# GuoleiSun/VSS-CFFM

Measured on AMD Instinct MI355X. Metric: clips/sec (fwd+bwd) CFFM-B1 480x480 T=4 hot path (CFFA+CFM, decoder_focal depth 2), higher is better.
Workload: dtype f32 in/out, f32 accumulate; MFMA operands: split-bf16 (hi+lo, ~2^-17) in the Linear GEMMs, f16 in QK^T/AV

## Files before the change

vss_cffm_amd/csrc/cffa_kernels.h:

```cpp
#pragma once
#include "cffm_common.h"

__device__ __forceinline__ void transpose_body(const float* __restrict__ src, float* __restrict__ dst,
                                               int rows, int cols, long src_bs, long dst_bs,
                                               const float* __restrict__ addend, int add_mod, int add_skip,
                                               float* __restrict__ copy_dst, int bx, int by, int bz) {
    __shared__ float tile[64][65];
    const int r0 = by * 64, c0 = bx * 64;
    const float* s = src + (long)bz * src_bs;
    float* d = dst + (long)bz * dst_bs;
    const int q = threadIdx.x & 15, p = threadIdx.x >> 4;
    const bool vin = (cols % 4 == 0) && (src_bs % 4 == 0) && (((uintptr_t)src & 15) == 0);
    const bool vout = (rows % 4 == 0) && (dst_bs % 4 == 0) && (((uintptr_t)dst & 15) == 0) && (((uintptr_t)addend & 15) == 0);
    const float* ad = (addend && (bz % add_mod) != add_skip) ? addend + (long)bz * dst_bs : nullptr;
    float* cp = (copy_dst && (bz % add_mod) != add_skip) ? copy_dst + (long)bz * src_bs : nullptr;
#pragma unroll
    for (int k = 0; k < 4; ++k) {
        const int r = r0 + p + 16 * k, c = c0 + 4 * q;
        f32x4 v = (f32x4){0.f, 0.f, 0.f, 0.f};
        if (r < rows) {
            if (vin && c + 3 < cols) {
                v = *(const f32x4*)(s + (long)r * cols + c);
                if (cp) *(f32x4*)(cp + (long)r * cols + c) = v;
            } else
                for (int e = 0; e < 4; ++e)
                    if (c + e < cols) { v[e] = s[(long)r * cols + c + e]; if (cp) cp[(long)r * cols + c + e] = v[e]; }
// ... 8 lines not shown
        f32x4 v;
#pragma unroll
        for (int e = 0; e < 4; ++e) v[e] = tile[cl][4 * q + e];
        if (c < cols) {
            if (vout && r + 3 < rows) *(f32x4*)(d + (long)c * rows + r) = ad ? v + *(const f32x4*)(ad + (long)c * rows + r) : v;
            else
                for (int e = 0; e < 4; ++e)
                    if (r + e < rows) d[(long)c * rows + r + e] = v[e] + (ad ? ad[(long)c * rows + r + e] : 0.f);
        }
    }
}
__global__ void __launch_bounds__(256) k_transpose(const float* __restrict__ src, float* __restrict__ dst,
                                                    int rows, int cols, long src_bs, long dst_bs,
                                                    const float* __restrict__ addend, int add_mod, int add_skip,
                                                    float* __restrict__ copy_dst = nullptr) {
    transpose_body(src, dst, rows, cols, src_bs, dst_bs, addend, add_mod, add_skip, copy_dst, blockIdx.x, blockIdx.y, blockIdx.z);
}

__device__ __forceinline__ float bil_tap(int r, int p) {
    if (p == r) return (11.f - 2.f * r) * (1.f / 12.f);
    if (p == r + 1) return (1.f + 2.f * r) * (1.f / 12.f);
    return 0.f;
}

__device__ __forceinline__ void cell_geom(int g, int& grp, int& u, int& v, int& wsg) {
    if (g == 0) { grp = 0; u = v = 0; wsg = 7; }
    else if (g == 1) { grp = 1; u = v = 0; wsg = 7; }
    else if (g < 6) { grp = 2; u = (g - 2) >> 1; v = (g - 2) & 1; wsg = 3; }
    else { grp = 3; u = (g - 6) / 3; v = (g - 6) % 3; wsg = 2; }
}

// ... 170 lines not shown

#define LNP_RSTRIDE 1216
#define LNP_TAIL_TGT (CFFM_WA + 1)
#define LNP_TAIL_REF (14 * CFFM_WA + 3)
#ifndef LNB_SPLIT
#define LNB_SPLIT 4
#endif
#ifndef LNB_WAVES
#define LNB_WAVES 4
#endif
#define LNB_THREADS (64 * LNB_WAVES)
#define LNB_PIX ((CFFM_WA + LNB_SPLIT * LNB_WAVES - 1) / (LNB_SPLIT * LNB_WAVES))

__device__ __forceinline__ float dot4(f32x4 a, f32x4 b) { return a[0] * b[0] + a[1] * b[1] + a[2] * b[2] + a[3] * b[3]; }

__global__ void __launch_bounds__(LNB_THREADS) k_ln_pool_bwd_tgt(Geo G, const float* __restrict__ x_tgt, long tgt_bs,
                                                                 const float* __restrict__ gamma, const float* __restrict__ beta,
                                                                 const float* __restrict__ M, const float* __restrict__ mean_in,
                                                                 const float* __restrict__ rstd_in, const float* __restrict__ dzall,
                                                                 const float* __restrict__ dres, float* __restrict__ dx_tgt, long dtgt_bs,
                                                                 float* __restrict__ rec) {
    __shared__ float red[LNB_WAVES][2][CFFM_C];
    __shared__ float sdM[CFFM_WA];
    __shared__ float sbs;
    const int s = blockIdx.x % LNB_SPLIT, wb = blockIdx.x / LNB_SPLIT;
    const int w = wb % G.nW, b = wb / G.nW;
    const int wy = w / G.gx, wx = w % G.gx;
    const int lane = threadIdx.x & 63, wave = wave_uniform(threadIdx.x >> 6);
    const float* xf = x_tgt + (long)b * tgt_bs;
    float* dxf = dx_tgt + (long)b * dtgt_bs;
    if (threadIdx.x < CFFM_WA) sdM[threadIdx.x] = 0.f;
    f32x4 xr[LNB_PIX], dzr[LNB_PIX], addr[LNB_PIX];
    float mur[LNB_PIX], rsr[LNB_PIX], m0[LNB_PIX];
#pragma unroll
    for (int k = 0; k < LNB_PIX; ++k) {
        const int i = s + LNB_SPLIT * (wave + LNB_WAVES * k);
        const int y = 7 * wy + i / 7, x = 7 * wx + i % 7;
        xr[k] = dzr[k] = addr[k] = (f32x4){0.f, 0.f, 0.f, 0.f};
        mur[k] = rsr[k] = m0[k] = 0.f;
        if (i < CFFM_WA && y < G.H0 && x < G.W0) {
// ... 26 lines not shown
        const f32x4 z = xh * gm + bt;
        const f32x4 dz = dzr[k] + m0[k] * dp;
        const float dm = wave_sum_hi(dot4(dp, z));
        if (lane == 63) sdM[i] = dm;
        ag += dz * xh;
        ab += dz;
        const f32x4 gz = dz * gm;
        const float m1 = wave_sum(gz[0] + gz[1] + gz[2] + gz[3]) * (1.f / CFFM_C);
        const float m2 = wave_sum(dot4(gz, xh)) * (1.f / CFFM_C);
        const f32x4 dx = (gz - m1 - xh * m2) * rs + addr[k];
        *(f32x4*)(dxf + pix * CFFM_C + 4 * lane) = dx;
    }
    *(f32x4*)(&red[wave][0][4 * lane]) = ag;
    *(f32x4*)(&red[wave][1][4 * lane]) = ab;
    __syncthreads();
    float* r = rec + (long)blockIdx.x * LNP_RSTRIDE;
    for (int e = threadIdx.x; e < 2 * CFFM_C; e += LNB_THREADS) {
        const int which = e / CFFM_C, ch = e % CFFM_C;
        float t = red[0][which][ch];
#pragma unroll
        for (int q = 1; q < LNB_WAVES; ++q) t += red[q][which][ch];
        r[e] = t;
    }
    if (threadIdx.x < CFFM_WA) r[2 * CFFM_C + threadIdx.x] = sdM[threadIdx.x];
    if (threadIdx.x == CFFM_WA) r[2 * CFFM_C + CFFM_WA] = sbs;
}

#define RB_MAXD 4
struct CffaRefBlocks {
    int n;
    const float* gamma[RB_MAXD];
    const float* beta[RB_MAXD];
    const float* M[RB_MAXD];
    const float* dzall[RB_MAXD];
    float* rec[RB_MAXD];
};
#define RB_LDS_BLOCK (14 * CFFM_C + 2 * 14 * CFFM_WA)
__host__ __device__ constexpr int cffa_ref_lds(int D) {
    return 4 * ((D * RB_LDS_BLOCK > LNB_WAVES * D * 2 * CFFM_C + 14 * D * CFFM_WA ? D * RB_LDS_BLOCK : LNB_WAVES * D * 2 * CFFM_C + 14 * D * CFFM_WA) + 4 * D + 4);
}
// ... 51 lines not shown
                    const float dm = wave_sum_hi(dot4(dp, z));
                    if (lane == 63) sdM[c * CFFM_WA + i] = dm;
                }
            ag[d] += dz * xh;
            ab[d] += dz;
            gz += dz * gm[d];
        }
        const float m1 = wave_sum(gz[0] + gz[1] + gz[2] + gz[3]) * (1.f / CFFM_C);
        const float m2 = wave_sum(dot4(gz, xh)) * (1.f / CFFM_C);
        const f32x4 dx = (gz - m1 - xh * m2) * rs + R.add[k];
        *(f32x4*)(dxf + pix * CFFM_C + 4 * lane) = dx;
    }
}

template <int D, bool ACC>
__global__ void __launch_bounds__(LNB_THREADS) k_ln_pool_bwd_ref(Geo G, const float* __restrict__ x_ref, long ref_bs, CffaRefBlocks Bk,
                                                                 const float* __restrict__ mean_in, const float* __restrict__ rstd_in,
                                                                 float* __restrict__ dx_ref, long dref_bs) {
    CFFM_DYN_SMEM(smem);
    float* sP = (float*)smem;
    float* sMm = sP + D * 14 * CFFM_C;
    float* red = (float*)smem;
    constexpr int body = D * (14 * CFFM_C + 14 * CFFM_WA), redn = LNB_WAVES * D * 2 * CFFM_C;
    float* sdM = (float*)smem + (body > redn ? body : redn);
    float* sbs = sdM + D * 14 * CFFM_WA;
    const int s = blockIdx.x % LNB_SPLIT, wb = blockIdx.x / LNB_SPLIT;
    const int w = wb % G.nW, b = wb / G.nW;
    const int wy = w / G.gx, wx = w % G.gx;
    const int lane = threadIdx.x & 63, wave = wave_uniform(threadIdx.x >> 6);
    for (int e = threadIdx.x; e < D * 14 * CFFM_WA; e += LNB_THREADS) {
        const int d = e / (14 * CFFM_WA), r = e % (14 * CFFM_WA);
        sMm[e] = Bk.M[d][CFFM_WA + r];
        sdM[e] = 0.f;
    }
    for (int r = wave; r < D * 14; r += LNB_WAVES) {
        const int d = r / 14, c = r % 14;
        *(f32x4*)(sP + r * CFFM_C + 4 * lane) = *(const f32x4*)(Bk.dzall[d] + ((long)b * G.RC + cell_row(G, wy, wx, 1 + c)) * CFFM_C + 4 * lane);
    }
    f32x4 gm[D], bt[D], ag[D], ab[D];
#pragma unroll
    for (int d = 0; d < D; ++d) {
// ... 23 lines not shown
    RefRows Ra, Rb;
    ln_pool_ref_load<ACC>(Ra, G, xb, dxb, mb, rb, s, wy, wx, lane, wave);
    ln_pool_ref_load<ACC>(Rb, G, xb + fr, dxb + fr, mb + G.HW, rb + G.HW, s, wy, wx, lane, wave);
    ln_pool_bwd_ref_frame<1, D>(G, Ra, dxb, sP, sMm, sdM, gm, bt, ag, ab, 1, s, wy, wx, lane, wave);
    ln_pool_ref_load<ACC>(Ra, G, xb + 2 * fr, dxb + 2 * fr, mb + 2 * G.HW, rb + 2 * G.HW, s, wy, wx, lane, wave);
    ln_pool_bwd_ref_frame<4, D>(G, Rb, dxb + fr, sP, sMm, sdM, gm, bt, ag, ab, 2, s, wy, wx, lane, wave);
    ln_pool_bwd_ref_frame<9, D>(G, Ra, dxb + 2 * fr, sP, sMm, sdM, gm, bt, ag, ab, 6, s, wy, wx, lane, wave);
    __syncthreads();
#pragma unroll
    for (int d = 0; d < D; ++d) {
        *(f32x4*)(red + ((wave * D + d) * 2 + 0) * CFFM_C + 4 * lane) = ag[d];
        *(f32x4*)(red + ((wave * D + d) * 2 + 1) * CFFM_C + 4 * lane) = ab[d];
    }
    __syncthreads();
    for (int d = 0; d < D; ++d) {
        float* r = Bk.rec[d] + (long)blockIdx.x * LNP_RSTRIDE;
        for (int e = threadIdx.x; e < 2 * CFFM_C; e += LNB_THREADS) {
            float t = red[(d * 2) * CFFM_C + e];
#pragma unroll
            for (int q = 1; q < LNB_WAVES; ++q) t += red[((q * D + d) * 2) * CFFM_C + e];
            r[e] = t;
        }
        for (int e = threadIdx.x; e < LNP_TAIL_REF; e += LNB_THREADS)
            r[2 * CFFM_C + e] = e < 14 * CFFM_WA ? sdM[d * 14 * CFFM_WA + e] : sbs[d * 4 + (e - 14 * CFFM_WA)];
    }
}
```

vss_cffm_amd/csrc/cffm_hip.hip:

```cpp
#include "cfm_attn_kernels.h"
#include "clip_kernels.h"
#include "rowops_kernels.h"
#include "gtc_kernels.h"
#include "gemm.h"
#include "segfuse_kernels.h"
#include "segloss_kernels.h"
#include "headfuse_kernels.h"
#include "kmeans_kernels.h"

#include <stdarg.h>
#include <stdio.h>

#include "../../include/cffm_hip.h"

static thread_local char g_err[512] = "";

static int fail(int code, const char* fmt, ...) {
    va_list ap;
    va_start(ap, fmt);
    vsnprintf(g_err, sizeof(g_err), fmt, ap);
    va_end(ap);
    return code;
}
#define CHECK_LAUNCH(name)                                                                        \
// ... 513 lines not shown
static float* g_redbuf[2] = {nullptr, nullptr};
static size_t g_red_floats_[2] = {0, 0};
static int g_red_parity = 0;
#define g_red g_redbuf[g_red_parity]
#define g_red_floats g_red_floats_[g_red_parity]
static struct { bool active; size_t bump; RedJobs jobs; } g_rq = {false, 0, {}};
static void redq_launch(RedJobs& J, hipStream_t st) {
    if (J.njob == 1) {
        CFFM_LAUNCH(k_reduce_records, ((J.total[0] + 63) / 64), (1024), 0, st, J.part[0], J.nblk[0], J.stride[0], J.total[0], J.segs[0]);
    } else if (J.njob > 1) {
        CFFM_LAUNCH(k_reduce_records_multi, ((unsigned)J.blk_end[J.njob - 1]), (1024), 0, st, J);
    }
    J.njob = 0;
}
static void redq_flush(hipStream_t st) { redq_launch(g_rq.jobs, st); }
struct RedScope {
    hipStream_t st;
    explicit RedScope(hipStream_t s) : st(s) { g_red_parity ^= 1; g_rq.active = true; g_rq.bump = 0; g_rq.jobs.njob = 0; }
    void finish() { redq_flush(st); g_rq.active = false; }
    void finish_on(hipStream_t other) { redq_flush(other); g_rq.active = false; }
    ~RedScope() { g_rq.active = false; g_rq.jobs.njob = 0; }
};
static float* red_scratch(size_t nfloats, hipStream_t st) {
    if (!g_rq.active) return lib_scratch(nfloats);
    nfloats = (nfloats + 63) / 64 * 64;
    if (g_rq.bump + nfloats > g_red_floats) {
#ifndef CFFM_EMU
        (void)hipDeviceSynchronize();
#endif
        redq_flush(st);
// ... 97 lines not shown
                             float* dx_ref, long dref_bs, int accum, hipStream_t st) {
    constexpr int lds = cffa_ref_lds(D);
#ifndef CFFM_EMU
    static bool granted = false;
    if (!granted && lds > 64 * 1024) {
        if (hipFuncSetAttribute((const void*)k_ln_pool_bwd_ref<D, false>, hipFuncAttributeMaxDynamicSharedMemorySize, lds) != hipSuccess ||
            hipFuncSetAttribute((const void*)k_ln_pool_bwd_ref<D, true>, hipFuncAttributeMaxDynamicSharedMemorySize, lds) != hipSuccess) return -1;
        granted = true;
    }
#endif
    if (accum) CFFM_LAUNCH((k_ln_pool_bwd_ref<D, true>), ((unsigned)cffa_rows(g)), (LNB_THREADS), lds, st, to_geo(g), x_ref, ref_bs, Bk, mean, rstd, dx_ref, dref_bs);
    else CFFM_LAUNCH((k_ln_pool_bwd_ref<D, false>), ((unsigned)cffa_rows(g)), (LNB_THREADS), lds, st, to_geo(g), x_ref, ref_bs, Bk, mean, rstd, dx_ref, dref_bs);
    return 0;
}
}
static int ln_pool_bwd_ref(const cffm_geom* g, const float* x_ref, long ref_bs, const CffaRefBlocks& Bk, const float* mean, const float* rstd,
                           float* dx_ref, long dref_bs, int accum, void* stream) {
    PROF(ST_LN_POOL_BWD_REF);
    hipStream_t st = (hipStream_t)stream;
    int rc = -1;
    switch (Bk.n) {
        case 1: rc = ln_pool_bwd_ref_d<1>(g, x_ref, ref_bs, Bk, mean, rstd, dx_ref, dref_bs, accum, st); break;
        case 2: rc = ln_pool_bwd_ref_d<2>(g, x_ref, ref_bs, Bk, mean, rstd, dx_ref, dref_bs, accum, st); break;
        case 3: rc = ln_pool_bwd_ref_d<3>(g, x_ref, ref_bs, Bk, mean, rstd, dx_ref, dref_bs, accum, st); break;
        case 4: rc = ln_pool_bwd_ref_d<4>(g, x_ref, ref_bs, Bk, mean, rstd, dx_ref, dref_bs, accum, st); break;
        default: break;
    }
    REQUIRE(!rc, "ln_pool_bwd_ref: bad block count %d or LDS grant failed", Bk.n);
    CHECK_LAUNCH("ln_pool_bwd_ref");
    return 0;
}
static void job_add(RedJobs& J, const float* part, int nblk, int stride, int total, const RedSegs& segs, hipStream_t st) {
    if (J.njob == RED_MAXJOB) redq_launch(J, st);
    const int j = J.njob++;
    J.part[j] = part; J.nblk[j] = nblk; J.stride[j] = stride; J.total[j] = total; J.segs[j] = segs;
    J.blk_end[j] = (j ? J.blk_end[j - 1] : 0) + (total + 63) / 64;
// ... 23 lines not shown
    if (g_scr4) { (void)hipDeviceSynchronize(); (void)hipFree(g_scr4); }
    if (hipMalloc((void**)&g_scr4, nfloats * sizeof(float)) != hipSuccess) g_scr4 = nullptr;
#endif
    g_scr4_floats = g_scr4 ? nfloats : 0;
    return g_scr4;
}
struct CffaSlot { float* dzall; float* rec; float* dM; };
static int cffa_slot(const cffm_geom* g, int slot, int nslots, CffaSlot* o) {
    const long a = up((long)g->B * g->RC * CFFM_C), b = up(2 * cffa_rows(g) * LNP_RSTRIDE), c = up(CFFM_NCELL * CFFM_WA);
    float* base = lib_scratch4((size_t)(a + b + c) * nslots);
    REQUIRE(base && slot >= 0 && slot < nslots, "cffa: scratch allocation failed");
    float* p = base + (a + b + c) * slot;
    o->dzall = p; o->rec = p + a; o->dM = p + a + b;
    return 0;
}
static int cffa_finish(const cffm_geom* g, int nslots, const cffm_block_params* params, const cffm_block_grads* grads, int first, int last,
                       const float* ws0, long ws_stride, const float* x_ref, long ref_bs, float* dx_ref, long dref_bs, int accum, void* stream,
                       RedJobs* extra = nullptr) {
    cffm_block_ws L;
    cffm_block_ws_layout(g, &L);
    hipStream_t st = (hipStream_t)stream;
    const long rows = cffa_rows(g);
    static_assert(PMB_MAXD == RB_MAXD, "one pooling-matrix launch per reference launch");
    for (int hi = first; hi >= last; hi -= RB_MAXD) {
        const int n = hi - last + 1 < RB_MAXD ? hi - last + 1 : RB_MAXD;
        CffaRefBlocks Bk;
        PoolWGN pw;
        RedJobs J;
        Bk.n = n; J.njob = 0;
        for (int d = 0; d < RB_MAXD; ++d) {
            const int i = hi - (d < n ? d : 0);
            CffaSlot S;
            TRY(cffa_slot(g, i, nslots, &S));
            Bk.gamma[d] = params[i].norm1_w; Bk.beta[d] = params[i].norm1_b; Bk.M[d] = ws0 + i * ws_stride + L.M;
            Bk.dzall[d] = S.dzall; Bk.rec[d] = S.rec + rows * LNP_RSTRIDE;
            pw.dM[d] = S.dM;
            for (int q = 0; q < 4; ++q) { pw.gw[d].w[q] = grads[i].pool_w[q]; pw.gw[d].b[q] = g_grad_pads ? grads[i].pool_b[q] : nullptr; }
        }
        const float* ws = ws0 + (long)hi * ws_stride;
        TRY(ln_pool_bwd_ref(g, x_ref, ref_bs, Bk, ws + L.mean1, ws + L.rstd1, dx_ref, dref_bs, accum || hi != first, stream));
        for (int d = 0; d < n; ++d) {
            const int i = hi - d;
            CffaSlot S;
            TRY(cffa_slot(g, i, nslots, &S));
            cffa_jobs(J, S.rec, rows, grads[i].norm1_w, grads[i].norm1_b, S.dM, grads[i].pool_b, st);
        }
        if (extra && hi - RB_MAXD < last) {
            for (int j = 0; j < extra->njob; ++j) job_add(J, extra->part[j], extra->nblk[j], extra->stride[j], extra->total[j], extra->segs[j], st);
            extra->njob = 0;
        }
        redq_launch(J, st);
        CHECK_LAUNCH("cffa reductions");
        {
            PROF(ST_POOLMAT);
            CFFM_LAUNCH(k_pool_matrix_bwd_n, (111, n), (64), 0, st, pw);
            CHECK_LAUNCH("pool_matrix_bwd");
        }
    }
    return 0;
}

int cffm_bias_assemble(const float* own, const float* ring, const float* const pool[4], float* bias, void* biasH, void* stream) {
    PROF(ST_BIAS_ASM);
    BiasTables t;
    t.own = own; t.ring = ring;
    for (int i = 0; i < 4; ++i) t.pool[i] = pool[i];
    const int n = CFFM_HEADS * CFFM_NQ_PAD * CFFM_NKEY_PAD;
    CFFM_LAUNCH(k_bias_assemble, ((n + 255) / 256), (256), 0, (hipStream_t)stream, t, bias, (h16*)biasH);
    CHECK_LAUNCH("bias_assemble");
    return 0;
}

// ... 629 lines not shown
                                   p->proj_b, p->fc1_b, p->fc2_b, p->norm2_w, p->norm2_b, ws + L.x1, nullptr, ws + L.mean2, ws + L.rstd2, ws + L.hraw,
                                   nullptr, ws + L.x2, ws + L.ao_t, ws + L.z2, ws + L.act, NP, stream));
        else
        TRY(cffm_mlp_fwd(ws + L.ao, x_tgt, tgt_bs, g->HW, wf + 768 * 256, wf + 768 * 256 + 256 * 256, wf + 768 * 256 + 256 * 256 + 1024 * 256,
                         p->proj_b, p->fc1_b, p->fc2_b, p->norm2_w, p->norm2_b, ws + L.x1, ws + L.z2, ws + L.mean2, ws + L.rstd2, ws + L.hraw,
                         ws + L.act, ws + L.x2, NP, stream));
        CHECK_LAUNCH("block_forward");
    }
    (void)scratch;
    return 0;
}

static int block_backward_impl(const cffm_geom* g, const cffm_block_params* p, const cffm_block_grads* gr,
                               const float* x_ref, long ref_bs, const float* x_tgt, long tgt_bs, const int* key_src,
                               const int* q_dst, const int* inv_ptr, const int* inv_idx, const float* ws, const float* dout,
                               float* dx_tgt, long dtgt_bs, float* scratch, int defer, int par, int slot, int nslots, void* stream);
#ifndef CFFM_EMU
static struct { bool has; RedJobs jobs; int parity; } g_tail = {false, {}, 0};
static int tail_flush(hipStream_t st) {
    if (!g_tail.has) return 0;
    g_tail.has = false;
    hipStream_t s3 = side_fork_take(st, 3);
    (void)hipStreamWaitEvent(s3, g_side.tail_order, 0);
    redq_launch(g_tail.jobs, s3);
    CHECK_LAUNCH("block_backward reductions");
    if (s3 != st) {
        side_record(s3, st, g_side.tail_done[g_tail.parity]);
        g_side.tail_pending[g_tail.parity] = true;
    }
    return 0;
}
// ... 6 lines not shown
    for (int i = 0; i < 2; ++i) g_side.dw_pending[i] = g_side.bias_pending[i] = g_side.tail_pending[i] = false;
#endif
}
int cffm_block_backward(const cffm_geom* g, const cffm_block_params* p, const cffm_block_grads* gr,
                        const float* x_ref, long ref_bs, const float* x_tgt, long tgt_bs, const int* key_src,
                        const int* q_dst, const int* inv_ptr, const int* inv_idx, const float* ws, const float* dout,
                        float* dx_ref, long dref_bs, int accum_ref, float* dx_tgt, long dtgt_bs, float* scratch, void* stream) {
    REQUIRE(x_ref && dx_ref, "block_backward: null");
    TRY(block_backward_impl(g, p, gr, x_ref, ref_bs, x_tgt, tgt_bs, key_src, q_dst, inv_ptr, inv_idx, ws, dout, dx_tgt, dtgt_bs, scratch, 0, 0, 0, 1,
                            stream));
    return cffa_finish(g, 1, p, gr, 0, 0, ws, 0, x_ref, ref_bs, dx_ref, dref_bs, accum_ref, stream);
}
static int block_backward_impl(const cffm_geom* g, const cffm_block_params* p, const cffm_block_grads* gr,
                               const float* x_ref, long ref_bs, const float* x_tgt, long tgt_bs, const int* key_src,
                               const int* q_dst, const int* inv_ptr, const int* inv_idx, const float* ws, const float* dout,
                               float* dx_tgt, long dtgt_bs, float* scratch, int defer, int par, int slot, int nslots, void* stream) {
    REQUIRE(g && p && gr && ws && dout && scratch, "block_backward: null");
    cffm_block_ws L;
    cffm_block_ws_layout(g, &L);
    const Scratch S = scratch_layout(g);
    const long NR = (long)g->B * g->RC, NP = (long)g->B * g->HW;
    par = (defer && par) ? 1 : 0;
    const long altb = S.alt, altact = altb + up(NP * CFFM_C), altqkv = altact + up((NP + 31) / 32 * 32 * CFFM_HID), altbias = altqkv + up(NR * 768);
    float* dx1 = scratch + (par ? altb : S.b);
    float* dz2 = scratch + S.dz2;
    float* dao = scratch + S.dao;
    float* dact = scratch + (par ? altact : S.dact);
    float* dqkv = scratch + (par ? altqkv : S.dqkv);
    const long NP32 = (NP + 31) / 32 * 32;
    float* dout_t = scratch + S.tf + (par ? S.tf_stride : 0);
    float* dx1_t = dout_t + up(NP32 * CFFM_C);
// ... 114 lines not shown
            const cffm_wgrad wgb[2] = {wg_qkv, wg_proj};
            const GemmTNPre preb[2] = {{0, 1, nullptr}, {0, 0, nullptr}};
            {
                void* stream = stream_b;
                PROF(ST_GEMM); PROF2(ST_G_DW);
                REQUIRE(!dw_group(wgb, preb, 2, sb, 320, dw_group_launched), "block_backward: weight-gradient gemm failed");
            }
            PROF(ST_ATTN_BWD);
            s1 = sb;
            TRY(attn_bwd_bias_sum(dbp, ng, dbiasT, (void*)s1));
            TRY(cffm_bias_scatter(dbiasT, gr->rpb_own, gr->rpb_ring, gr->rpb_pool, (void*)s1));
        }
        return 0;
    };
    const bool side_late = stream_dw && one_group;
    if (!side_late) TRY(side_b());
    if (!side_late && (!one_group || dx_tgt == dout)) side_join(sa, st, 0);
#ifndef CFFM_EMU
    if (g_side.dw_pending[par ^ 1] && g_side.dw_dout[par ^ 1] == dx_tgt) {
        side_wait(st, g_side.dw_done[par ^ 1]);
        g_side.dw_pending[par ^ 1] = false;
    }
#endif
    TRY(ln_pool_bwd_tgt(g, x_tgt, tgt_bs, p->norm1_w, p->norm1_b, ws + L.M, ws + L.mean1, ws + L.rstd1, dzall, dx1, dx_tgt, dtgt_bs, cffa.rec,
                        stream));
    if (side_late) TRY(side_b());
#ifndef CFFM_EMU
    if (defer && sb != st && s1 != st && g_side.on) {
        if (g_tail.has) TRY(tail_flush(st));
        side_fork_mark(st, 3);
        if (s1 != sb) side_order(s1, sb);
        (void)hipEventRecord(g_side.tail_order, sb);
        g_tail.has = true; g_tail.jobs = g_rq.jobs; g_tail.parity = g_red_parity;
        g_rq.jobs.njob = 0; g_rq.active = false;
        g_side.dw_pending[par] = true;
        g_side.dw_dout[par] = dout;
        side_record(s1, st, g_side.bias_done[par]);
        g_side.bias_pending[par] = true;
        return 0;
    }
#endif
// ... 451 lines not shown
    REQUIRE(hipMemcpyAsync(y_rows, blk0 + (long)(depth - 1) * L.total + L.x2, (size_t)g->B * img * sizeof(float), hipMemcpyDeviceToDevice,
                           (hipStream_t)stream) == hipSuccess, "layer_forward_rows: copy failed");
#endif
    return 0;
}
int cffm_layer_backward_rows(const cffm_geom* g, int depth, const cffm_block_params* params, const cffm_block_grads* grads,
                             const float* x_rows, const float* dy_rows, float* dx_rows, const int* key_src, const int* q_dst,
                             const int* inv_ptr, const int* inv_idx, const float* saved, float* scratch, void* stream) {
    REQUIRE(g && params && grads && x_rows && dy_rows && dx_rows && saved && scratch && depth >= 1, "layer_backward_rows: bad arguments");
    cffm_block_ws L;
    cffm_block_ws_layout(g, &L);
    const Scratch S = scratch_layout(g);
    const long HW = g->HW, img = HW * CFFM_C;
    const float* blk0 = saved + up((long)g->B * 4 * img);
    tail_reset();
    for (int i = depth - 1; i >= 0; --i) {
        const float* ws = blk0 + (long)i * L.total;
        const float* tgt = (i == 0) ? x_rows + 3 * img : blk0 + (long)(i - 1) * L.total + L.x2;
        const long tgt_bs = (i == 0) ? 4 * img : img;
        float* dtgt = (i == 0) ? dx_rows + 3 * img : scratch + (((depth - i) & 1) ? S.a2 : S.a);
        const long dtgt_bs = (i == 0) ? 4 * img : img;
        const float* dout = (i == depth - 1) ? dy_rows : scratch + (((depth - 1 - i) & 1) ? S.a2 : S.a);
        TRY(block_backward_impl(g, &params[i], &grads[i], x_rows, 4 * img, tgt, tgt_bs, key_src, q_dst, inv_ptr, inv_idx, ws, dout, dtgt, dtgt_bs,
                                scratch, 1, (depth - 1 - i) & 1, i, depth, stream));
    }
    RedJobs* tail_jobs = nullptr;
#ifndef CFFM_EMU
    if (g_tail.has) {
        g_tail.has = false;
        tail_jobs = &g_tail.jobs;
    }
#endif
    TRY(cffa_finish(g, depth, params, grads, depth - 1, 0, blk0, L.total, x_rows, 4 * img, dx_rows, 4 * img, 0, stream, tail_jobs));
    side_join_all((hipStream_t)stream);
    return 0;
}

static int layer_forward_impl(const cffm_geom* g, int depth, const cffm_block_params* params, const float* x_nchw,
                              float* y_tgt_nchw, long y_bs, float* y_full, const int* key_src, const int* q_dst, float* saved,
                              float* scratch, void* stream) {
    REQUIRE(g && params && x_nchw && y_tgt_nchw && saved && scratch && depth >= 1, "layer_forward: bad arguments");
    cffm_block_ws L;
    cffm_block_ws_layout(g, &L);
    const long HW = g->HW, img = HW * CFFM_C;
    float* xs = saved;
    float* blk0 = saved + up((long)g->B * 4 * img);
    hipStream_t st = (hipStream_t)stream;
    side_init(st);
// ... 192 lines not shown
                               const int* q_dst, const int* inv_ptr, const int* inv_idx, const float* saved, float* scratch,
                               int first_block, int last_block, void* stream) {
    REQUIRE(g && params && grads && dy_tgt_nchw && dx_nchw && saved && scratch && depth >= 1, "layer_backward: bad arguments");
    REQUIRE(first_block < depth && last_block >= 0 && first_block >= last_block, "layer_backward: bad block range %d..%d of %d", first_block,
            last_block, depth);
    cffm_block_ws L;
    cffm_block_ws_layout(g, &L);
    const Scratch S = scratch_layout(g);
    const long HW = g->HW, img = HW * CFFM_C;
    const float* xs = saved;
    const float* blk0 = saved + up((long)g->B * 4 * img);
    float* dxs = scratch + S.dxs;
    REQUIRE(dy_bs >= img, "layer_backward: dy batch stride %ld < %ld", dy_bs, img);
    if (first_block == depth - 1) TRY(cffm_transpose(dy_tgt_nchw, scratch + S.a, g->B, CFFM_C, (int)HW, dy_bs, img, stream));
    tail_reset();
    for (int i = first_block; i >= last_block; --i) {
        const float* ws = blk0 + (long)i * L.total;
        const float* tgt = (i == 0) ? xs + 3 * img : blk0 + (long)(i - 1) * L.total + L.x2;
        const long tgt_bs = (i == 0) ? 4 * img : img;
        float* dcur = scratch + (((depth - 1 - i) & 1) ? S.a2 : S.a);
        float* dtgt = (i == 0) ? dxs + 3 * img : scratch + (((depth - i) & 1) ? S.a2 : S.a);
        const long dtgt_bs = (i == 0) ? 4 * img : img;
        TRY(block_backward_impl(g, &params[i], &grads[i], xs, 4 * img, tgt, tgt_bs, key_src, q_dst, inv_ptr, inv_idx, ws, dcur, dtgt, dtgt_bs, scratch,
                                1, (depth - 1 - i) & 1, i, depth, stream));
    }
    RedJobs* tail_jobs = nullptr;
#ifndef CFFM_EMU
    if (last_block == 0 && g_tail.has) {
        g_tail.has = false;
        tail_jobs = &g_tail.jobs;
    }
#endif
    TRY(cffa_finish(g, depth, params, grads, first_block, last_block, blk0, L.total, xs, 4 * img, dxs, 4 * img, first_block != depth - 1, stream, tail_jobs));
    if (last_block == 0) TRY(transpose_add(dxs, dx_nchw, g->B * 4, (int)HW, CFFM_C, img, img, dy_full, 4, 3, stream));
    TRY(tail_flush((hipStream_t)stream));
    side_join_all((hipStream_t)stream);
    return 0;
}
int cffm_layer_backward_range(const cffm_geom* g, int depth, const cffm_block_params* params, const cffm_block_grads* grads,
                              const float* dy_tgt_nchw, long dy_bs, float* dx_nchw, const int* key_src, const int* q_dst,
                              const int* inv_ptr, const int* inv_idx, const float* saved, float* scratch, int first_block,
                              int last_block, void* stream) {
    return layer_backward_impl(g, depth, params, grads, dy_tgt_nchw, dy_bs, nullptr, dx_nchw, key_src, q_dst, inv_ptr, inv_idx, saved,
                               scratch, first_block, last_block, stream);
}
int cffm_layer_backward_full(const cffm_geom* g, int depth, const cffm_block_params* params, const cffm_block_grads* grads,
                             const float* dy_full_nchw, float* dx_nchw, const int* key_src, const int* q_dst, const int* inv_ptr,
                             const int* inv_idx, const float* saved, float* scratch, int first_block, int last_block, void* stream) {
    REQUIRE(g && dy_full_nchw && dy_full_nchw != dx_nchw, "layer_backward_full: bad arguments");
// ... 84 lines not shown
```

vss_cffm_amd/csrc/rowops_kernels.h:

```cpp
#pragma once
#include "cffm_common.h"
#include "cffa_kernels.h"
#include "panel_kernels.h"

struct BiasTables {
    const float* own;
    const float* ring;
    const float* pool[4];
};
struct BiasTablesG {
    float* own;
    float* ring;
    float* pool[4];
};

__device__ __forceinline__ int bias_locate(int h, int q, int n, int& off) {
    const int qi = q / 7, qj = q % 7;
    if (n < 49) {
        const int ki = n / 7, kj = n % 7;
        off = ((qi - ki + 6) * 13 + (qj - kj + 6)) * CFFM_HEADS + h;
        return 0;
    }
    if (n < 181) {
        off = (h * 49 + q) * 132 + (n - 49);
// ... 68 lines not shown
    if (a.pack == 2) return;
    long e = (long)(bx - a.nbias - 1) * 256 + threadIdx.x;
    long off = 0;
#pragma unroll
    for (int k = 0; k < 4; ++k) {
        if (e >= off && e < off + n4[k]) ((f32x4*)a.w_s[d])[e] = split4_pack(((const f32x4*)a.w[d][k])[e - off]);
        off += n4[k];
    }
}
__global__ void __launch_bounds__(256) k_param_prep(PrepArgs a) { param_prep_body(a, blockIdx.x, blockIdx.y); }
struct TrArgs { const float* src; float* dst; int rows, cols; long src_bs, dst_bs; int add_mod, add_skip; float* copy_dst; int gx, gy, gz; };
__global__ void __launch_bounds__(256) k_transpose_prep(TrArgs T, PrepArgs a, int pnx) {
    const int nt = T.gx * T.gy * T.gz;
    int b = blockIdx.x;
    if (b < nt) {
        transpose_body(T.src, T.dst, T.rows, T.cols, T.src_bs, T.dst_bs, nullptr, T.add_mod, T.add_skip, T.copy_dst, b % T.gx, (b / T.gx) % T.gy,
                       b / (T.gx * T.gy));
        return;
    }
    b -= nt;
    param_prep_body(a, b % pnx, b / pnx);
}

__global__ void __launch_bounds__(256) k_bias_scatter(const float* __restrict__ dbiasT, BiasTablesG g) {
    const int e = blockIdx.x * 256 + threadIdx.x;
    const int n_own = 169 * CFFM_HEADS, n_ring = CFFM_HEADS * 49 * 132;
    if (e < n_ring) {
        const int n = e % 132, q = (e / 132) % 49, h = e / (132 * 49);
        g.ring[e] = dbiasT[((long)h * CFFM_NKEY_PAD + 49 + n) * CFFM_NQ_PAD + q];
    }
    if (blockIdx.x * 256 + 255 < n_ring) return;
    const int j = (e - n_ring) & 15;
// ... 135 lines not shown
struct RedJobs {
    int njob;
    int blk_end[RED_MAXJOB];
    const float* part[RED_MAXJOB];
    int nblk[RED_MAXJOB], stride[RED_MAXJOB], total[RED_MAXJOB];
    RedSegs segs[RED_MAXJOB];
};
__global__ void __launch_bounds__(1024) k_reduce_records_multi(RedJobs J) {
    __shared__ float red[64][64];
    int blk = blockIdx.x, j = 0;
#pragma unroll
    for (int q = 0; q < RED_MAXJOB - 1; ++q)
        if (q + 1 < J.njob && blk >= J.blk_end[q]) j = q + 1;
    if (j > 0) blk -= J.blk_end[j - 1];
    reduce_records_body(J.part[j], J.nblk[j], J.stride[j], J.total[j], J.segs[j], blk, red);
}

#define COLSUM_ROWS 32
__global__ void __launch_bounds__(256) k_colsum_partial(const float* __restrict__ a, long nrows, int ncol, float* __restrict__ part) {
    const long r0 = (long)blockIdx.x * COLSUM_ROWS;
    for (int c4 = threadIdx.x; c4 < ncol / 4; c4 += 256) {
        f32x4 acc = (f32x4){0.f, 0.f, 0.f, 0.f};
#pragma unroll
        for (int k0 = 0; k0 < COLSUM_ROWS; k0 += 8) {
            f32x4 v[8];
#pragma unroll
            for (int k = 0; k < 8; ++k) v[k] = (r0 + k0 + k < nrows) ? ((const f32x4*)(a + (r0 + k0 + k) * ncol))[c4] : (f32x4){0.f, 0.f, 0.f, 0.f};
            acc += ((v[0] + v[1]) + (v[2] + v[3])) + ((v[4] + v[5]) + (v[6] + v[7]));
        }
        ((f32x4*)(part + (long)blockIdx.x * ncol))[c4] = acc;
// ... 187 lines not shown
```

Measured before the change: 2890.

## Fuse last-block LN-pool target backward with reference pass and reductions with output transpose

Result: no change. 2930, median of 6 (+1.4%).

```diff
diff --git a/vss_cffm_amd/csrc/cffa_kernels.h b/vss_cffm_amd/csrc/cffa_kernels.h
--- a/vss_cffm_amd/csrc/cffa_kernels.h
+++ b/vss_cffm_amd/csrc/cffa_kernels.h
@@ -4,12 +4,13 @@
 __device__ __forceinline__ void transpose_body(const float* __restrict__ src, float* __restrict__ dst,
                                                int rows, int cols, long src_bs, long dst_bs,
                                                const float* __restrict__ addend, int add_mod, int add_skip,
-                                               float* __restrict__ copy_dst, int bx, int by, int bz) {
-    __shared__ float tile[64][65];
+                                               float* __restrict__ copy_dst, int bx, int by, int bz,
+                                               float (*tile)[65], int tid, bool live = true) {
     const int r0 = by * 64, c0 = bx * 64;
     const float* s = src + (long)bz * src_bs;
     float* d = dst + (long)bz * dst_bs;
-    const int q = threadIdx.x & 15, p = threadIdx.x >> 4;
+    const int q = tid & 15, p = tid >> 4;
+    if (!live) rows = cols = 0;
     const bool vin = (cols % 4 == 0) && (src_bs % 4 == 0) && (((uintptr_t)src & 15) == 0);
     const bool vout = (rows % 4 == 0) && (dst_bs % 4 == 0) && (((uintptr_t)dst & 15) == 0) && (((uintptr_t)addend & 15) == 0);
     const float* ad = (addend && (bz % add_mod) != add_skip) ? addend + (long)bz * dst_bs : nullptr;
@@ -48,7 +49,8 @@
                                                     int rows, int cols, long src_bs, long dst_bs,
                                                     const float* __restrict__ addend, int add_mod, int add_skip,
                                                     float* __restrict__ copy_dst = nullptr) {
-    transpose_body(src, dst, rows, cols, src_bs, dst_bs, addend, add_mod, add_skip, copy_dst, blockIdx.x, blockIdx.y, blockIdx.z);
+    __shared__ float tile[64][65];
+    transpose_body(src, dst, rows, cols, src_bs, dst_bs, addend, add_mod, add_skip, copy_dst, blockIdx.x, blockIdx.y, blockIdx.z, tile, threadIdx.x);
 }
 
 __device__ __forceinline__ float bil_tap(int r, int p) {
@@ -249,16 +251,17 @@
 
 __device__ __forceinline__ float dot4(f32x4 a, f32x4 b) { return a[0] * b[0] + a[1] * b[1] + a[2] * b[2] + a[3] * b[3]; }
 
-__global__ void __launch_bounds__(LNB_THREADS) k_ln_pool_bwd_tgt(Geo G, const float* __restrict__ x_tgt, long tgt_bs,
-                                                                 const float* __restrict__ gamma, const float* __restrict__ beta,
-                                                                 const float* __restrict__ M, const float* __restrict__ mean_in,
-                                                                 const float* __restrict__ rstd_in, const float* __restrict__ dzall,
-                                                                 const float* __restrict__ dres, float* __restrict__ dx_tgt, long dtgt_bs,
-                                                                 float* __restrict__ rec) {
-    __shared__ float red[LNB_WAVES][2][CFFM_C];
-    __shared__ float sdM[CFFM_WA];
-    __shared__ float sbs;
-    const int s = blockIdx.x % LNB_SPLIT, wb = blockIdx.x / LNB_SPLIT;
+#define LNB_TGT_LDS (LNB_WAVES * 2 * CFFM_C + 64 + 4)
+__device__ __forceinline__ void ln_pool_bwd_tgt_body(const Geo& G, const float* __restrict__ x_tgt, long tgt_bs,
+                                                     const float* __restrict__ gamma, const float* __restrict__ beta,
+                                                     const float* __restrict__ M, const float* __restrict__ mean_in,
+                                                     const float* __restrict__ rstd_in, const float* __restrict__ dzall,
+                                                     const float* __restrict__ dres, float* __restrict__ dx_tgt, long dtgt_bs,
+                                                     float* __restrict__ rec, int blk, float* lds) {
+    float (*red)[2][CFFM_C] = (float (*)[2][CFFM_C])lds;
+    float* sdM = lds + LNB_WAVES * 2 * CFFM_C;
+    float& sbs = lds[LNB_WAVES * 2 * CFFM_C + 64];
+    const int s = blk % LNB_SPLIT, wb = blk / LNB_SPLIT;
     const int w = wb % G.nW, b = wb / G.nW;
     const int wy = w / G.gx, wx = w % G.gx;
     const int lane = threadIdx.x & 63, wave = wave_uniform(threadIdx.x >> 6);
@@ -315,7 +318,7 @@
     *(f32x4*)(&red[wave][0][4 * lane]) = ag;
     *(f32x4*)(&red[wave][1][4 * lane]) = ab;
     __syncthreads();
-    float* r = rec + (long)blockIdx.x * LNP_RSTRIDE;
+    float* r = rec + (long)blk * LNP_RSTRIDE;
     for (int e = threadIdx.x; e < 2 * CFFM_C; e += LNB_THREADS) {
         const int which = e / CFFM_C, ch = e % CFFM_C;
         float t = red[0][which][ch];
@@ -325,6 +328,15 @@
     }
     if (threadIdx.x < CFFM_WA) r[2 * CFFM_C + threadIdx.x] = sdM[threadIdx.x];
     if (threadIdx.x == CFFM_WA) r[2 * CFFM_C + CFFM_WA] = sbs;
+}
+__global__ void __launch_bounds__(LNB_THREADS) k_ln_pool_bwd_tgt(Geo G, const float* __restrict__ x_tgt, long tgt_bs,
+                                                                 const float* __restrict__ gamma, const float* __restrict__ beta,
+                                                                 const float* __restrict__ M, const float* __restrict__ mean_in,
+                                                                 const float* __restrict__ rstd_in, const float* __restrict__ dzall,
+                                                                 const float* __restrict__ dres, float* __restrict__ dx_tgt, long dtgt_bs,
+                                                                 float* __restrict__ rec) {
+    __shared__ __attribute__((aligned(16))) float lds[LNB_TGT_LDS];
+    ln_pool_bwd_tgt_body(G, x_tgt, tgt_bs, gamma, beta, M, mean_in, rstd_in, dzall, dres, dx_tgt, dtgt_bs, rec, blockIdx.x, lds);
 }
 
 #define RB_MAXD 4
@@ -406,17 +418,16 @@
 }
 
 template <int D, bool ACC>
-__global__ void __launch_bounds__(LNB_THREADS) k_ln_pool_bwd_ref(Geo G, const float* __restrict__ x_ref, long ref_bs, CffaRefBlocks Bk,
-                                                                 const float* __restrict__ mean_in, const float* __restrict__ rstd_in,
-                                                                 float* __restrict__ dx_ref, long dref_bs) {
-    CFFM_DYN_SMEM(smem);
+__device__ __forceinline__ void ln_pool_bwd_ref_body(const Geo& G, const float* __restrict__ x_ref, long ref_bs, const CffaRefBlocks& Bk,
+                                                     const float* __restrict__ mean_in, const float* __restrict__ rstd_in,
+                                                     float* __restrict__ dx_ref, long dref_bs, int blk, char* smem) {
     float* sP = (float*)smem;
     float* sMm = sP + D * 14 * CFFM_C;
     float* red = (float*)smem;
     constexpr int body = D * (14 * CFFM_C + 14 * CFFM_WA), redn = LNB_WAVES * D * 2 * CFFM_C;
     float* sdM = (float*)smem + (body > redn ? body : redn);
     float* sbs = sdM + D * 14 * CFFM_WA;
-    const int s = blockIdx.x % LNB_SPLIT, wb = blockIdx.x / LNB_SPLIT;
+    const int s = blk % LNB_SPLIT, wb = blk / LNB_SPLIT;
     const int w = wb % G.nW, b = wb / G.nW;
     const int wy = w / G.gx, wx = w % G.gx;
     const int lane = threadIdx.x & 63, wave = wave_uniform(threadIdx.x >> 6);
@@ -470,7 +481,7 @@
     }
     __syncthreads();
     for (int d = 0; d < D; ++d) {
-        float* r = Bk.rec[d] + (long)blockIdx.x * LNP_RSTRIDE;
+        float* r = Bk.rec[d] + (long)blk * LNP_RSTRIDE;
         for (int e = threadIdx.x; e < 2 * CFFM_C; e += LNB_THREADS) {
             float t = red[(d * 2) * CFFM_C + e];
 #pragma unroll
@@ -481,3 +492,37 @@
             r[2 * CFFM_C + e] = e < 14 * CFFM_WA ? sdM[d * 14 * CFFM_WA + e] : sbs[d * 4 + (e - 14 * CFFM_WA)];
     }
 }
+template <int D, bool ACC>
+__global__ void __launch_bounds__(LNB_THREADS) k_ln_pool_bwd_ref(Geo G, const float* __restrict__ x_ref, long ref_bs, CffaRefBlocks Bk,
+                                                                 const float* __restrict__ mean_in, const float* __restrict__ rstd_in,
+                                                                 float* __restrict__ dx_ref, long dref_bs) {
+    CFFM_DYN_SMEM(smem);
+    ln_pool_bwd_ref_body<D, ACC>(G, x_ref, ref_bs, Bk, mean_in, rstd_in, dx_ref, dref_bs, blockIdx.x, smem);
+}
+
+#ifndef LNB_LAST_INTERLEAVE
+#define LNB_LAST_INTERLEAVE 0
+#endif
+struct CffaTgtPass {
+    const float *x_tgt, *gamma, *beta, *M, *mean, *rstd, *dzall, *dres;
+    float *dx_tgt, *rec;
+    long tgt_bs, dtgt_bs;
+};
+static_assert(cffa_ref_lds(1) >= 4 * LNB_TGT_LDS, "the target role lives in the reference role's LDS");
+template <int D, bool ACC>
+__global__ void __launch_bounds__(LNB_THREADS) k_ln_pool_bwd_last(Geo G, CffaTgtPass T, const float* __restrict__ x_ref, long ref_bs, CffaRefBlocks Bk,
+                                                                  const float* __restrict__ mean_in, const float* __restrict__ rstd_in,
+                                                                  float* __restrict__ dx_ref, long dref_bs) {
+    CFFM_DYN_SMEM(smem);
+    const int rows = gridDim.x >> 1;
+#if LNB_LAST_INTERLEAVE
+    const bool ref = (blockIdx.x & 1) == 0;
+    const int blk = blockIdx.x >> 1;
+#else
+    const bool ref = (int)blockIdx.x < rows;
+    const int blk = ref ? blockIdx.x : blockIdx.x - rows;
+#endif
+    (void)rows;
+    if (ref) ln_pool_bwd_ref_body<D, ACC>(G, x_ref, ref_bs, Bk, mean_in, rstd_in, dx_ref, dref_bs, blk, smem);
+    else ln_pool_bwd_tgt_body(G, T.x_tgt, T.tgt_bs, T.gamma, T.beta, T.M, T.mean, T.rstd, T.dzall, T.dres, T.dx_tgt, T.dtgt_bs, T.rec, blk, (float*)smem);
+}
diff --git a/vss_cffm_amd/csrc/cffm_hip.hip b/vss_cffm_amd/csrc/cffm_hip.hip
--- a/vss_cffm_amd/csrc/cffm_hip.hip
+++ b/vss_cffm_amd/csrc/cffm_hip.hip
@@ -551,6 +551,19 @@
     J.njob = 0;
 }
 static void redq_flush(hipStream_t st) { redq_launch(g_rq.jobs, st); }
+static int redq_launch_transpose(RedJobs& J, const TransposeJob& T, hipStream_t st) {
+#ifndef CFFM_EMU
+    static bool granted = false;
+    if (!granted) {
+        if (hipFuncSetAttribute((const void*)k_reduce_transpose, hipFuncAttributeMaxDynamicSharedMemorySize, RT_LDS) != hipSuccess) return -1;
+        granted = true;
+    }
+#endif
+    const int nred = J.njob ? J.blk_end[J.njob - 1] : 0;
+    CFFM_LAUNCH(k_reduce_transpose, ((unsigned)(nred + (T.ntile + RT_TILES - 1) / RT_TILES)), (1024), RT_LDS, st, J, nred, T);
+    J.njob = 0;
+    return 0;
+}
 struct RedScope {
     hipStream_t st;
     explicit RedScope(hipStream_t s) : st(s) { g_red_parity ^= 1; g_rq.active = true; g_rq.bump = 0; g_rq.jobs.njob = 0; }
@@ -678,12 +691,38 @@
     return 0;
 }
 }
+extern "C++" {
+template <int D>
+static int ln_pool_bwd_last_d(const cffm_geom* g, const CffaTgtPass& T, const float* x_ref, long ref_bs, const CffaRefBlocks& Bk, const float* mean,
+                              const float* rstd, float* dx_ref, long dref_bs, int accum, hipStream_t st) {
+    constexpr int lds = cffa_ref_lds(D);
+#ifndef CFFM_EMU
+    static bool granted = false;
+    if (!granted && lds > 64 * 1024) {
+        if (hipFuncSetAttribute((const void*)k_ln_pool_bwd_last<D, false>, hipFuncAttributeMaxDynamicSharedMemorySize, lds) != hipSuccess ||
+            hipFuncSetAttribute((const void*)k_ln_pool_bwd_last<D, true>, hipFuncAttributeMaxDynamicSharedMemorySize, lds) != hipSuccess) return -1;
+        granted = true;
+    }
+#endif
+    const unsigned grid = (unsigned)(2 * cffa_rows(g));
+    if (accum) CFFM_LAUNCH((k_ln_pool_bwd_last<D, true>), (grid), (LNB_THREADS), lds, st, to_geo(g), T, x_ref, ref_bs, Bk, mean, rstd, dx_ref, dref_bs);
+    else CFFM_LAUNCH((k_ln_pool_bwd_last<D, false>), (grid), (LNB_THREADS), lds, st, to_geo(g), T, x_ref, ref_bs, Bk, mean, rstd, dx_ref, dref_bs);
+    return 0;
+}
+}
 static int ln_pool_bwd_ref(const cffm_geom* g, const float* x_ref, long ref_bs, const CffaRefBlocks& Bk, const float* mean, const float* rstd,
-                           float* dx_ref, long dref_bs, int accum, void* stream) {
+                           float* dx_ref, long dref_bs, int accum, void* stream, const CffaTgtPass* tgt = nullptr) {
     PROF(ST_LN_POOL_BWD_REF);
     hipStream_t st = (hipStream_t)stream;
     int rc = -1;
-    switch (Bk.n) {
+    if (tgt) switch (Bk.n) {
+        case 1: rc = ln_pool_bwd_last_d<1>(g, *tgt, x_ref, ref_bs, Bk, mean, rstd, dx_ref, dref_bs, accum, st); break;
+        case 2: rc = ln_pool_bwd_last_d<2>(g, *tgt, x_ref, ref_bs, Bk, mean, rstd, dx_ref, dref_bs, accum, st); break;
+        case 3: rc = ln_pool_bwd_last_d<3>(g, *tgt, x_ref, ref_bs, Bk, mean, rstd, dx_ref, dref_bs, accum, st); break;
+        case 4: rc = ln_pool_bwd_last_d<4>(g, *tgt, x_ref, ref_bs, Bk, mean, rstd, dx_ref, dref_bs, accum, st); break;
+        default: break;
+    }
+    else switch (Bk.n) {
         case 1: rc = ln_pool_bwd_ref_d<1>(g, x_ref, ref_bs, Bk, mean, rstd, dx_ref, dref_bs, accum, st); break;
         case 2: rc = ln_pool_bwd_ref_d<2>(g, x_ref, ref_bs, Bk, mean, rstd, dx_ref, dref_bs, accum, st); break;
         case 3: rc = ln_pool_bwd_ref_d<3>(g, x_ref, ref_bs, Bk, mean, rstd, dx_ref, dref_bs, accum, st); break;
@@ -737,9 +776,12 @@
     o->dzall = p; o->rec = p + a; o->dM = p + a + b;
     return 0;
 }
+#ifndef CFFA_SHARED_TAIL
+#define CFFA_SHARED_TAIL 3
+#endif
 static int cffa_finish(const cffm_geom* g, int nslots, const cffm_block_params* params, const cffm_block_grads* grads, int first, int last,
                        const float* ws0, long ws_stride, const float* x_ref, long ref_bs, float* dx_ref, long dref_bs, int accum, void* stream,
-                       RedJobs* extra = nullptr) {
+                       RedJobs* extra = nullptr, const CffaTgtPass* tgt = nullptr, const TransposeJob* out = nullptr) {
     cffm_block_ws L;
     cffm_block_ws_layout(g, &L);
     hipStream_t st = (hipStream_t)stream;
@@ -761,7 +803,7 @@
             for (int q = 0; q < 4; ++q) { pw.gw[d].w[q] = grads[i].pool_w[q]; pw.gw[d].b[q] = g_grad_pads ? grads[i].pool_b[q] : nullptr; }
         }
         const float* ws = ws0 + (long)hi * ws_stride;
-        TRY(ln_pool_bwd_ref(g, x_ref, ref_bs, Bk, ws + L.mean1, ws + L.rstd1, dx_ref, dref_bs, accum || hi != first, stream));
+        TRY(ln_pool_bwd_ref(g, x_ref, ref_bs, Bk, ws + L.mean1, ws + L.rstd1, dx_ref, dref_bs, accum || hi != first, stream, hi == first ? tgt : nullptr));
         for (int d = 0; d < n; ++d) {
             const int i = hi - d;
             CffaSlot S;
@@ -772,13 +814,18 @@
             for (int j = 0; j < extra->njob; ++j) job_add(J, extra->part[j], extra->nblk[j], extra->stride[j], extra->total[j], extra->segs[j], st);
             extra->njob = 0;
         }
-        redq_launch(J, st);
+        const bool with_out = out && hi - RB_MAXD < last;
+        if (with_out && (CFFA_SHARED_TAIL & 2)) REQUIRE(!redq_launch_transpose(J, *out, st), "cffa reductions: LDS grant failed");
+        else redq_launch(J, st);
         CHECK_LAUNCH("cffa reductions");
         {
             PROF(ST_POOLMAT);
             CFFM_LAUNCH(k_pool_matrix_bwd_n, (111, n), (64), 0, st, pw);
             CHECK_LAUNCH("pool_matrix_bwd");
         }
+        if (with_out && !(CFFA_SHARED_TAIL & 2))
+            TRY(transpose_add(out->src, out->dst, out->ntile / (out->tx * out->ty), out->rows, out->cols, out->src_bs, out->dst_bs, out->addend,
+                              out->add_mod, out->add_skip, stream));
     }
     return 0;
 }
@@ -1438,7 +1485,8 @@
 static int block_backward_impl(const cffm_geom* g, const cffm_block_params* p, const cffm_block_grads* gr,
                                const float* x_ref, long ref_bs, const float* x_tgt, long tgt_bs, const int* key_src,
                                const int* q_dst, const int* inv_ptr, const int* inv_idx, const float* ws, const float* dout,
-                               float* dx_tgt, long dtgt_bs, float* scratch, int defer, int par, int slot, int nslots, void* stream);
+                               float* dx_tgt, long dtgt_bs, float* scratch, int defer, int par, int slot, int nslots, void* stream,
+                               CffaTgtPass* tgt_later = nullptr);
 #ifndef CFFM_EMU
 static struct { bool has; RedJobs jobs; int parity; } g_tail = {false, {}, 0};
 static int tail_flush(hipStream_t st) {
@@ -1475,7 +1523,8 @@
 static int block_backward_impl(const cffm_geom* g, const cffm_block_params* p, const cffm_block_grads* gr,
                                const float* x_ref, long ref_bs, const float* x_tgt, long tgt_bs, const int* key_src,
                                const int* q_dst, const int* inv_ptr, const int* inv_idx, const float* ws, const float* dout,
-                               float* dx_tgt, long dtgt_bs, float* scratch, int defer, int par, int slot, int nslots, void* stream) {
+                               float* dx_tgt, long dtgt_bs, float* scratch, int defer, int par, int slot, int nslots, void* stream,
+                               CffaTgtPass* tgt_later) {
     REQUIRE(g && p && gr && ws && dout && scratch, "block_backward: null");
     cffm_block_ws L;
     cffm_block_ws_layout(g, &L);
@@ -1620,7 +1669,7 @@
         return 0;
     };
     const bool side_late = stream_dw && one_group;
-    if (!side_late) TRY(side_b());
+    if (!side_late || tgt_later) TRY(side_b());
     if (!side_late && (!one_group || dx_tgt == dout)) side_join(sa, st, 0);
 #ifndef CFFM_EMU
     if (g_side.dw_pending[par ^ 1] && g_side.dw_dout[par ^ 1] == dx_tgt) {
@@ -1628,9 +1677,15 @@
         g_side.dw_pending[par ^ 1] = false;
     }
 #endif
-    TRY(ln_pool_bwd_tgt(g, x_tgt, tgt_bs, p->norm1_w, p->norm1_b, ws + L.M, ws + L.mean1, ws + L.rstd1, dzall, dx1, dx_tgt, dtgt_bs, cffa.rec,
-                        stream));
-    if (side_late) TRY(side_b());
+    if (tgt_later) {
+        CffaTgtPass& T = *tgt_later;
+        T.x_tgt = x_tgt; T.tgt_bs = tgt_bs; T.gamma = p->norm1_w; T.beta = p->norm1_b; T.M = ws + L.M; T.mean = ws + L.mean1; T.rstd = ws + L.rstd1;
+        T.dzall = dzall; T.dres = dx1; T.dx_tgt = dx_tgt; T.dtgt_bs = dtgt_bs; T.rec = cffa.rec;
+    } else {
+        TRY(ln_pool_bwd_tgt(g, x_tgt, tgt_bs, p->norm1_w, p->norm1_b, ws + L.M, ws + L.mean1, ws + L.rstd1, dzall, dx1, dx_tgt, dtgt_bs, cffa.rec,
+                            stream));
+        if (side_late) TRY(side_b());
+    }
 #ifndef CFFM_EMU
     if (defer && sb != st && s1 != st && g_side.on) {
         if (g_tail.has) TRY(tail_flush(st));
@@ -2112,6 +2167,7 @@
     const long HW = g->HW, img = HW * CFFM_C;
     const float* blk0 = saved + up((long)g->B * 4 * img);
     tail_reset();
+    CffaTgtPass tgt_pass;
     for (int i = depth - 1; i >= 0; --i) {
         const float* ws = blk0 + (long)i * L.total;
         const float* tgt = (i == 0) ? x_rows + 3 * img : blk0 + (long)(i - 1) * L.total + L.x2;
@@ -2120,7 +2176,7 @@
         const long dtgt_bs = (i == 0) ? 4 * img : img;
         const float* dout = (i == depth - 1) ? dy_rows : scratch + (((depth - 1 - i) & 1) ? S.a2 : S.a);
         TRY(block_backward_impl(g, &params[i], &grads[i], x_rows, 4 * img, tgt, tgt_bs, key_src, q_dst, inv_ptr, inv_idx, ws, dout, dtgt, dtgt_bs,
-                                scratch, 1, (depth - 1 - i) & 1, i, depth, stream));
+                                scratch, 1, (depth - 1 - i) & 1, i, depth, stream, (CFFA_SHARED_TAIL & 1) && i == 0 ? &tgt_pass : nullptr));
     }
     RedJobs* tail_jobs = nullptr;
 #ifndef CFFM_EMU
@@ -2129,7 +2185,7 @@
         tail_jobs = &g_tail.jobs;
     }
 #endif
-    TRY(cffa_finish(g, depth, params, grads, depth - 1, 0, blk0, L.total, x_rows, 4 * img, dx_rows, 4 * img, 0, stream, tail_jobs));
+    TRY(cffa_finish(g, depth, params, grads, depth - 1, 0, blk0, L.total, x_rows, 4 * img, dx_rows, 4 * img, 0, stream, tail_jobs, (CFFA_SHARED_TAIL & 1) ? &tgt_pass : nullptr));
     side_join_all((hipStream_t)stream);
     return 0;
 }
@@ -2352,6 +2408,7 @@
     REQUIRE(dy_bs >= img, "layer_backward: dy batch stride %ld < %ld", dy_bs, img);
     if (first_block == depth - 1) TRY(cffm_transpose(dy_tgt_nchw, scratch + S.a, g->B, CFFM_C, (int)HW, dy_bs, img, stream));
     tail_reset();
+    CffaTgtPass tgt_pass;
     for (int i = first_block; i >= last_block; --i) {
         const float* ws = blk0 + (long)i * L.total;
         const float* tgt = (i == 0) ? xs + 3 * img : blk0 + (long)(i - 1) * L.total + L.x2;
@@ -2360,7 +2417,7 @@
         float* dtgt = (i == 0) ? dxs + 3 * img : scratch + (((depth - i) & 1) ? S.a2 : S.a);
         const long dtgt_bs = (i == 0) ? 4 * img : img;
         TRY(block_backward_impl(g, &params[i], &grads[i], xs, 4 * img, tgt, tgt_bs, key_src, q_dst, inv_ptr, inv_idx, ws, dcur, dtgt, dtgt_bs, scratch,
-                                1, (depth - 1 - i) & 1, i, depth, stream));
+                                1, (depth - 1 - i) & 1, i, depth, stream, (CFFA_SHARED_TAIL & 1) && i == last_block ? &tgt_pass : nullptr));
     }
     RedJobs* tail_jobs = nullptr;
 #ifndef CFFM_EMU
@@ -2369,8 +2426,12 @@
         tail_jobs = &g_tail.jobs;
     }
 #endif
-    TRY(cffa_finish(g, depth, params, grads, first_block, last_block, blk0, L.total, xs, 4 * img, dxs, 4 * img, first_block != depth - 1, stream, tail_jobs));
-    if (last_block == 0) TRY(transpose_add(dxs, dx_nchw, g->B * 4, (int)HW, CFFM_C, img, img, dy_full, 4, 3, stream));
+    TransposeJob out;
+    out.src = dxs; out.dst = dx_nchw; out.addend = dy_full; out.src_bs = out.dst_bs = img;
+    out.rows = (int)HW; out.cols = CFFM_C; out.add_mod = 4; out.add_skip = 3;
+    out.tx = (CFFM_C + 63) / 64; out.ty = (int)((HW + 63) / 64); out.ntile = out.tx * out.ty * g->B * 4;
+    TRY(cffa_finish(g, depth, params, grads, first_block, last_block, blk0, L.total, xs, 4 * img, dxs, 4 * img, first_block != depth - 1, stream, tail_jobs,
+                    (CFFA_SHARED_TAIL & 1) ? &tgt_pass : nullptr, last_block == 0 ? &out : nullptr));
     TRY(tail_flush((hipStream_t)stream));
     side_join_all((hipStream_t)stream);
     return 0;
diff --git a/vss_cffm_amd/csrc/rowops_kernels.h b/vss_cffm_amd/csrc/rowops_kernels.h
--- a/vss_cffm_amd/csrc/rowops_kernels.h
+++ b/vss_cffm_amd/csrc/rowops_kernels.h
@@ -106,8 +106,9 @@
     const int nt = T.gx * T.gy * T.gz;
     int b = blockIdx.x;
     if (b < nt) {
+        __shared__ float tile[64][65];
         transpose_body(T.src, T.dst, T.rows, T.cols, T.src_bs, T.dst_bs, nullptr, T.add_mod, T.add_skip, T.copy_dst, b % T.gx, (b / T.gx) % T.gy,
-                       b / (T.gx * T.gy));
+                       b / (T.gx * T.gy), tile, threadIdx.x);
         return;
     }
     b -= nt;
@@ -273,6 +274,34 @@
         if (q + 1 < J.njob && blk >= J.blk_end[q]) j = q + 1;
     if (j > 0) blk -= J.blk_end[j - 1];
     reduce_records_body(J.part[j], J.nblk[j], J.stride[j], J.total[j], J.segs[j], blk, red);
+}
+
+#define RT_TILES 4
+#define RT_LDS (RT_TILES * 64 * 65 * 4)
+static_assert(RT_LDS >= 64 * 64 * 4, "the reduction's LDS");
+struct TransposeJob {
+    const float* src; float* dst; const float* addend;
+    long src_bs, dst_bs;
+    int rows, cols, add_mod, add_skip;
+    int tx, ty, ntile;
+};
+__global__ void __launch_bounds__(1024) k_reduce_transpose(RedJobs J, int nred, TransposeJob T) {
+    CFFM_DYN_SMEM(smem);
+    if ((int)blockIdx.x < nred) {
+        int blk = blockIdx.x, j = 0;
+#pragma unroll
+        for (int q = 0; q < RED_MAXJOB - 1; ++q)
+            if (q + 1 < J.njob && blk >= J.blk_end[q]) j = q + 1;
+        if (j > 0) blk -= J.blk_end[j - 1];
+        reduce_records_body(J.part[j], J.nblk[j], J.stride[j], J.total[j], J.segs[j], blk, (float (*)[64])smem);
+        return;
+    }
+    const int sub = wave_uniform(threadIdx.x >> 8);
+    const int t = ((int)blockIdx.x - nred) * RT_TILES + sub;
+    const bool live = t < T.ntile;
+    const int tl = live ? t : 0;
+    transpose_body(T.src, T.dst, T.rows, T.cols, T.src_bs, T.dst_bs, T.addend, T.add_mod, T.add_skip, nullptr, tl % T.tx, (tl / T.tx) % T.ty,
+                   tl / (T.tx * T.ty), (float (*)[65])smem + 64 * sub, threadIdx.x & 255, live);
 }
 
 #define COLSUM_ROWS 32
```
